# ChrisTho23/DrakeGPT

Measured on AMD Instinct MI355X. Metric: training tokens/sec (fwd+bwd+AdamW), higher is better.
Workload: dtype bf16; 1 GPU; TransformerLM_scaled: V=80 C=384 T=256 heads=6 layers=6 dropout=0.2; fwd+bwd+AdamW; hipGraph=on; batch_per_gpu=64, global_batch=64, seq_len=256, parallelism=dp1, dp_gradient_buckets=1, params=10800464

## Files before the change

### drakegpt_amd/csrc/chain.hip

```cpp
#include "common.h"
#include <stdlib.h>

typedef __attribute__((address_space(1))) const void* gptr_t;
typedef __attribute__((address_space(3))) void* lptr_t;

#define CH_C 384
#define CH_ROWS 64
#define CH_STAGE_B 24576
#define CH_STAGE_A 4096
#define CH_STAGE (CH_STAGE_B + CH_STAGE_A)
#define CH_NST 4
#define CH_ARES (CH_NST * CH_STAGE)
#define CH_KS (CH_C / 32)

struct ChainP {
    const char* o;
    const float* x;
    const char* wproj; const float* bproj;
    float* x1;
    const float* ln2w; const float* ln2b; float* mean2; float* rstd2; bf16_t* h2;
    const char* w1; const float* b1; bf16_t* f; unsigned char* bits;
    const char* w2; const float* b2;
    float* x2; bf16_t* x2b;
    const float* ln1w; const float* ln1b; float* mean1; float* rstd1; bf16_t* h1;
// ... 470 lines not shown
                stamp(4 + 2 * c);
            }
        }
        if (HAS_FFN2) {
            piece(4 * KS, MODE != 4, HAS_QKV, false, true);
            stamp(11);
            if (p.dbg == 4 || p.dbg == 5) { if (LN_FFN2) __builtin_amdgcn_s_barrier(); }
            else {
                float xv[2][3][8];
                residual_epilogue(xv, row0, MODE == 1 ? p.b2 : nullptr, p.x1, key_ffn, MODE != 1 ? p.x2 : nullptr, p.x2b);
                if (LN_FFN2)
                    layernorm(xv, (float*)(lds + (g & (CH_NST - 1)) * CH_STAGE + CH_STAGE_B), row0, p.mean1, p.rstd1, p.h1);
            }
        }
        stamp(12);
        if (HAS_QKV) {
            for (int c = 0; c < 3; ++c) {
                piece(KS, false, c < 2, MODE == 0 && c == 0);
                stamp(13 + 2 * c);
                if (p.dbg == 4 || p.dbg == 5) continue;
                const int lo = opaque_lane(), fr = lo & 15, fg = lo >> 4, col_l = wn * 96 + (fg & 1) * 16 + (fg >> 1) * 8;
#pragma unroll
                for (int q = 0; q < 3; ++q) {
                    const int col = c * C + col_l + 32 * q;
#pragma unroll
                    for (int i = 0; i < 2; ++i) {
                        const int64_t row = row0 + wm * 32 + i * 16 + fr;
                        float v[8];
                        take(i, q, v);
                        bf16x8 o;
#pragma unroll
                        for (int e = 0; e < 8; ++e) o[e] = (bf16_t)v[e];
                        if (p.dbg != 6) *(bf16x8*)(p.qkv + row0 * (3 * C) + mad24(wm * 32 + i * 16 + fr, 3 * C, col)) = o;
                    }
                }
                stamp(14 + 2 * c);
            }
        }
        stamp(19);
        __builtin_amdgcn_s_barrier();
        stamp(20);
    }
}

struct PackOne { const unsigned short* src; unsigned short* dst; int N, K; int64_t ld; };
__global__ __launch_bounds__(256) void pack_chain_kernel(const int64_t* __restrict__ desc, int n_desc, PackOne one) {
    const unsigned short* src = one.src;
    unsigned short* dst = one.dst;
    int K = one.K;
    int64_t ld = one.ld;
    int k = blockIdx.x;
    if (desc) {
        int d = 0;
        for (int i = 1; i < n_desc; ++i)
            if ((int64_t)blockIdx.x >= desc[i * 6 + 4]) d = i;
        const int64_t* D = desc + d * 6;
        src = (const unsigned short*)D[0]; dst = (unsigned short*)D[1]; K = (int)D[3]; ld = D[5];
        k = (int)((int64_t)blockIdx.x - D[4]);
    }
    const int KT = K / 32, c = k / KT, t = k % KT;
    if (!(KT & 1)) {
        const int half = t & 1, t0 = t - half;
        const int64_t k0 = k - half;
#pragma unroll
        for (int u = 0; u < 6; ++u) {
            const int idx = threadIdx.x + 256 * u, line = 96 * half + (idx >> 4), hi = (idx >> 3) & 1, j = idx & 7;
            const int slot = (hi * 4 + (j & 3)) ^ (line & 7);
            const int row = c * 384 + line + 192 * hi, col = t0 * 32 + 8 * j;
            *(u32x4*)(dst + ((k0 + (j >> 2)) * 1536 + line * 8 + slot) * 8) = *(const u32x4*)(src + (int64_t)row * ld + col);
        }
        return;
    }
#pragma unroll
    for (int u = 0; u < 6; ++u) {
        const int idx = threadIdx.x + 256 * u, line = idx >> 3, slot = idx & 7, ls = slot ^ (line & 7);
        const int row = c * 384 + line + 192 * (ls >> 2), col = t * 32 + 8 * (ls & 3);
        *(u32x4*)(dst + ((int64_t)k * 1536 + idx) * 8) = *(const u32x4*)(src + (int64_t)row * ld + col);
    }
}

extern "C" int dg_pack_chain_weights(const void* w, int64_t ld, void* packed, int N, int K, void* stream) {
    if (!w || !packed || N <= 0 || K <= 0 || N % 384 || K % 32 || ld < K || ld % 8 || !dg_aligned16(w) || !dg_aligned16(packed)) return DG_ERR_ARG;
    PackOne one{(const unsigned short*)w, (unsigned short*)packed, N, K, ld};
    hipLaunchKernelGGL(pack_chain_kernel, dim3((N / 384) * (K / 32)), dim3(256), 0, (hipStream_t)stream, (const int64_t*)nullptr, 0, one);
    DG_LAUNCH_CHECK();
    return DG_OK;
}

extern "C" int dg_pack_chain_weights_batched(const int64_t* desc, int n_desc, int total_stages, void* stream) {
    if (!desc || n_desc <= 0 || total_stages <= 0) return DG_ERR_ARG;
    PackOne one{nullptr, nullptr, 0, 0, 0};
    hipLaunchKernelGGL(pack_chain_kernel, dim3(total_stages), dim3(256), 0, (hipStream_t)stream, desc, n_desc, one);
    DG_LAUNCH_CHECK();
    return DG_OK;
}

__global__ __launch_bounds__(256) void l2_warm_kernel(const char* __restrict__ p, int64_t n_lines, float* __restrict__ sink) {
    const int j = (int)blockIdx.x >> 3, per = (int)gridDim.x >> 3;
    float acc = 0.f;
    for (int64_t i = (int64_t)j * 256 + threadIdx.x; i < n_lines; i += (int64_t)per * 256) acc += *(const float*)(p + i * 128);
    if (acc == 123.456f && sink) sink[0] = acc;
}

extern "C" int dg_l2_warm(const void* p, int64_t bytes, void* stream) {
    if (!p || bytes <= 0 || (((uintptr_t)p) & 127)) return DG_ERR_ARG;
    hipLaunchKernelGGL(l2_warm_kernel, dim3(256), dim3(256), 0, (hipStream_t)stream, (const char*)p, bytes / 128, (float*)nullptr);
    DG_LAUNCH_CHECK();
    return DG_OK;
// ... 62 lines not shown
```

### drakegpt_amd/csrc/cross_entropy.hip

```cpp
#include "common.h"
#include <float.h>
#include <type_traits>

struct CeOpt { float eps, zeta; };
struct CeIgn { int64_t ignore_index; const float* inv_count; };
template <typename... O> struct CePack {
    static constexpr bool OPT = dg_pack_has<CeOpt, O...>::value, IGN = dg_pack_has<CeIgn, O...>::value;
    CeOpt opt;
    CeIgn ign;
    __device__ __forceinline__ explicit CePack(O... o) : opt(dg_pack_get(CeOpt{0.f, 0.f}, o...)), ign(dg_pack_get(CeIgn{0, nullptr}, o...)) {}
};
__device__ __forceinline__ float ce_objective(float mx, float logs, float xt, float sd, int V, CeOpt opt) {
    const float lse = mx + logs;
    return logs + (1.f - opt.eps) * (mx - xt) + opt.eps / (float)V * sd + opt.zeta * lse * lse;
}
template <bool OPT, bool IGN>
__device__ __forceinline__ float ce_row_loss(float mx, float logs, float xt, float sd, int V, CeOpt opt) {
    return OPT ? ce_objective(mx, logs, xt, sd, V, opt) : IGN ? logs + (mx - xt) : mx + logs - xt;
}
__device__ __forceinline__ float ce_pscale(float mx, float logs, CeOpt opt) { return 1.f + 2.f * opt.zeta * (mx + logs); }
template <bool OPT> __device__ __forceinline__ float ce_inv(float mx, float logs, float s, CeOpt opt) {
    return OPT ? ce_pscale(mx, logs, opt) / s : 1.f / s;
}
template <bool OPT> __device__ __forceinline__ float ce_unif(int V, CeOpt opt) { return OPT ? opt.eps / (float)V : 0.f; }
// ... 89 lines not shown
    }
    if (!ok) return;
    if (IGN && skip) {
        if (sub == 0) loss_rows[row] = 0.f;
        if (dlogits) {
#pragma unroll
            for (int k = 0; k < 8; ++k)
                if (sub + 16 * k < (int)ldd) dlogits[(int64_t)row * ldd + sub + 16 * k] = from_f32<TD>(0.f);
        }
        return;
    }
    const int64_t t = ce_clamp_target(targets[row], V);
    if (sub == 0) loss_rows[row] = ce_row_loss<OPT, IGN>(mx, logf(s), x[t], sd, V, p.opt);
    if (dlogits) {
        TD* d = dlogits + (int64_t)row * ldd;
        const float inv = ce_inv<OPT>(mx, logf(s), s, p.opt), unif = ce_unif<OPT>(V, p.opt);
        if (gs_dev) grad_scale *= gs_dev[0];
        if (IGN) grad_scale *= p.ign.inv_count[0];
#pragma unroll
        for (int k = 0; k < 8; ++k) {
            const int i = sub + 16 * k;
            if (i < (int)ldd) d[i] = from_f32<TD>(i >= V ? 0.f : ce_grad<OPT>(v[k] * inv, i == (int)t, unif, p.opt, grad_scale));
        }
    }
}

struct CeFuse {
    float* colsum_part; int64_t part_stride; int rows_per;
    float* loss_part; unsigned* counter; float* loss_out; float loss_scale;
};
#define CEF_THREADS 1024
#define CEF_RG (CEF_THREADS / 16)
template <typename TD, typename... O>
__global__ __launch_bounds__(CEF_THREADS) void cross_entropy_small_fused_kernel(const float* __restrict__ logits, int64_t ldl, const int64_t* __restrict__ targets,
                                                                        float* __restrict__ loss_rows, TD* __restrict__ dlogits, int64_t ldd,
                                                                        float grad_scale, int M, int V, CeFuse fz, O... o) {
    const CePack<O...> p(o...);
    constexpr bool OPT = p.OPT, IGN = p.IGN;
    __shared__ float red[CEF_RG][128];
    __shared__ float lred[CEF_RG];
    __shared__ unsigned last_flag;
    const int tid = threadIdx.x, sub = tid & 15, rg = tid >> 4;
    const int m_begin = blockIdx.x * fz.rows_per;
    int m_end = m_begin + fz.rows_per; if (m_end > M) m_end = M;
    float cacc[8];
#pragma unroll
    for (int k = 0; k < 8; ++k) cacc[k] = 0.f;
    float lsum = 0.f;
    if (IGN) grad_scale *= p.ign.inv_count[0];
    for (int r0 = m_begin; r0 < m_end; r0 += CEF_RG) {
        const int row = r0 + rg;
        const bool ok = row < m_end;
        const float* x = logits + (int64_t)(ok ? row : m_begin) * ldl;
        const bool skip = IGN && ok && targets[row] == p.ign.ignore_index;
        float v[8];
        float mx = -INFINITY;
#pragma unroll
        for (int k = 0; k < 8; ++k) {
            const int i = sub + 16 * k;
            v[k] = i < V ? (IGN && skip ? 0.f : x[i]) : -INFINITY;
            mx = fmaxf(mx, v[k]);
        }
#pragma unroll
        for (int o = 8; o > 0; o >>= 1) mx = fmaxf(mx, __shfl_xor(mx, o, 64));
        float s = 0.f, sd = 0.f;
#pragma unroll
        for (int k = 0; k < 8; ++k) {
            if (OPT && sub + 16 * k < V) sd += mx - v[k];
            v[k] = expf(v[k] - mx); s += v[k];
        }
#pragma unroll
        for (int sh = 8; sh > 0; sh >>= 1) s += __shfl_xor(s, sh, 64);
        if (OPT) {
#pragma unroll
            for (int sh = 8; sh > 0; sh >>= 1) sd += __shfl_xor(sd, sh, 64);
        }
        if (!ok) continue;
        if (IGN && skip) {
            if (sub == 0) loss_rows[row] = 0.f;
#pragma unroll
            for (int k = 0; k < 8; ++k)
                if (sub + 16 * k < (int)ldd) dlogits[(int64_t)row * ldd + sub + 16 * k] = from_f32<TD>(0.f);
            continue;
        }
        const int64_t t = ce_clamp_target(targets[row], V);
        const float lr = ce_row_loss<OPT, IGN>(mx, logf(s), x[t], sd, V, p.opt);
        if (sub == 0) { loss_rows[row] = lr; lsum += lr; }
        TD* d = dlogits + (int64_t)row * ldd;
        const float inv = ce_inv<OPT>(mx, logf(s), s, p.opt), unif = ce_unif<OPT>(V, p.opt);
#pragma unroll
        for (int k = 0; k < 8; ++k) {
            const int i = sub + 16 * k;
            const float gk = i >= V ? 0.f : ce_grad<OPT>(v[k] * inv, i == (int)t, unif, p.opt, grad_scale);
            cacc[k] += gk;
            if (i < (int)ldd) d[i] = from_f32<TD>(gk);
        }
    }
#pragma unroll
    for (int k = 0; k < 8; ++k) red[rg][sub + 16 * k] = cacc[k];
    if (sub == 0) lred[rg] = lsum;
    __syncthreads();
    if (fz.colsum_part && tid < V) {
        float c = 0.f;
#pragma unroll 8
        for (int r = 0; r < CEF_RG; ++r) c += red[r][tid];
        fz.colsum_part[(int64_t)blockIdx.x * fz.part_stride + tid] = c;
    }
    if (!fz.loss_out) return;
    if (tid == 0) {
        float b = 0.f;
#pragma unroll 8
        for (int r = 0; r < CEF_RG; ++r) b += lred[r];
        __hip_atomic_store(fz.loss_part + blockIdx.x, b, __ATOMIC_RELAXED, __HIP_MEMORY_SCOPE_AGENT);
        asm volatile("s_waitcnt vmcnt(0)" ::: "memory");
        const unsigned prev = __hip_atomic_fetch_add(fz.counter, 1u, __ATOMIC_RELAXED, __HIP_MEMORY_SCOPE_AGENT);
        last_flag = prev == gridDim.x - 1 ? 1u : 0u;
    }
    __syncthreads();
    if (!last_flag) return;
    __builtin_amdgcn_fence(__ATOMIC_ACQUIRE, "workgroup");
    float* sh = &red[0][0];
    for (int i = tid; i < (int)gridDim.x; i += CEF_THREADS) sh[i] = __hip_atomic_load(fz.loss_part + i, __ATOMIC_RELAXED, __HIP_MEMORY_SCOPE_AGENT);
    __syncthreads();
    if (tid == 0) {
        float tot = 0.f;
        for (int i = 0; i < (int)gridDim.x; ++i) tot += sh[i];
        fz.loss_out[0] = IGN ? tot * (fz.loss_scale * p.ign.inv_count[0]) : tot * fz.loss_scale;
        __hip_atomic_store(fz.counter, 0u, __ATOMIC_RELAXED, __HIP_MEMORY_SCOPE_AGENT);
    }
}

#define CE_BLOCK 1024
#define CE_MAXK 52
__device__ __forceinline__ float ce_block_max(const float* red) {
    __syncthreads();
    float mx = red[0];
#pragma unroll
    for (int k = 1; k < 16; ++k) mx = fmaxf(mx, red[k]);
    __syncthreads();
    return mx;
}
struct CeSums { float s, sd; };
template <bool OPT> __device__ __forceinline__ CeSums ce_block_sums(const float* red, const float* red2) {
    __syncthreads();
    float s = red[0], sd = 0.f;
#pragma unroll
    for (int k = 1; k < 16; ++k) s += red[k];
    if (OPT) {
        sd = red2[0];
#pragma unroll
        for (int k = 1; k < 16; ++k) sd += red2[k];
    }
    return CeSums{s, sd};
}

template <typename TD, typename TL = float, typename... O>
__global__ __launch_bounds__(CE_BLOCK) void cross_entropy_row_kernel(const TL* logits, int64_t ldl, const int64_t* __restrict__ targets,
                                                                      float* __restrict__ loss_rows, TD* dlogits, int64_t ldd,
                                                                      float grad_scale, const float* __restrict__ gs_dev, int M, int V, O... o) {
    const CePack<O...> p(o...);
    constexpr bool OPT = p.OPT, IGN = p.IGN;
    __shared__ float red[16];
    __shared__ float red2[OPT ? 16 : 1];
    const int tid = threadIdx.x, lane = tid & 63, w = tid >> 6;
    const int row = blockIdx.x;
    const TL* x = logits + (int64_t)row * ldl;
    int64_t t = targets[row];
    if (IGN && t == p.ign.ignore_index)
        return ce_zero_row(loss_rows, dlogits, ldd, row, tid, CE_BLOCK);
    float v[CE_MAXK];
    float mx = -INFINITY;
    t = ce_clamp_target(t, V);
    const float xt = (float)x[t];
#pragma unroll
    for (int k = 0; k < CE_MAXK; ++k) {
        const int i = k * CE_BLOCK + tid;
        v[k] = i < V ? (float)x[i] : -INFINITY;
        mx = fmaxf(mx, v[k]);
    }
// ... 280 lines not shown
```

### drakegpt_amd/csrc/elementwise.hip

```cpp
#include "common.h"

__global__ void state_advance_kernel(uint32_t* st) { st[2] += 1u; }

extern "C" int dg_state_advance(uint32_t* rng_state, void* stream) {
    if (!rng_state) return DG_ERR_ARG;
    hipLaunchKernelGGL(state_advance_kernel, dim3(1), dim3(1), 0, (hipStream_t)stream, rng_state);
    DG_LAUNCH_CHECK();
    return DG_OK;
}

__global__ void batch_gather_kernel(const int64_t* __restrict__ corpus, int64_t n_corpus,
                                    const int64_t* __restrict__ off, int64_t* __restrict__ x,
                                    int64_t* __restrict__ y, int B, int T) {
    int64_t i = (int64_t)blockIdx.x * blockDim.x + threadIdx.x;
    if (i >= (int64_t)B * T) return;
    int b = (int)(i / T), t = (int)(i % T);
    int64_t o = off[b] + t;
    int64_t o1 = o + 1;
    if (o < 0) o = 0; if (o >= n_corpus) o = n_corpus - 1;
    if (o1 < 0) o1 = 0; if (o1 >= n_corpus) o1 = n_corpus - 1;
    x[i] = corpus[o];
    y[i] = corpus[o1];
}

// ... 18 lines not shown
    const int cv = C / VEC;
    int64_t total = M * cv;
    const int64_t* off = nullptr;
    if (GATHER) {
        uint32_t row = 0;
        if (bs.ctl) {
            const uint32_t n_rows = bs.ctl[1];
            row = bs.step_state[2] - bs.ctl[0];
            if (row >= n_rows) row = n_rows ? n_rows - 1 : 0;
        }
        off = bs.offsets + (int64_t)row * bs.B;
    }
    (void)total;
    const int lane = threadIdx.x & 63;
    const int64_t wave0 = ((int64_t)blockIdx.x * blockDim.x + threadIdx.x) >> 6, nwaves = ((int64_t)gridDim.x * blockDim.x) >> 6;
    for (int64_t m = wave0; m < M; m += nwaves) {
        const uint32_t mu = (uint32_t)__builtin_amdgcn_readfirstlane((int)m);
        const uint32_t bq = mu / (uint32_t)T;
        const int t = (int)(mu - bq * (uint32_t)T);
        int64_t v;
        if (GATHER) {
            int64_t o = off[bq] + t, o1 = o + 1;
            if (o < 0) o = 0; if (o >= bs.n_corpus) o = bs.n_corpus - 1;
            if (o1 < 0) o1 = 0; if (o1 >= bs.n_corpus) o1 = bs.n_corpus - 1;
            v = bs.corpus[o];
            if (lane == 0) { bs.x_ids[m] = v; bs.y_ids[m] = bs.corpus[o1]; }
        } else {
            v = idx[m];
        }
        v = v < 0 ? 0 : (v >= V ? V - 1 : v);
      for (int j = lane; j < cv; j += 64) {
        const int c = j * VEC;
        if (onehot) {
            if (VEC == 4 && j * 8 < ld_onehot) {
                bf16x8 o;
#pragma unroll
                for (int e = 0; e < 8; ++e) o[e] = (bf16_t)((int64_t)(j * 8 + e) == v ? 1.f : 0.f);
                *(bf16x8*)(onehot + m * ld_onehot + j * 8) = o;
            }
        }
        if (VEC == 4) {
            f32x4 a = *(const f32x4*)(tok + v * C + c);
            if (pos) a += *(const f32x4*)(pos + (int64_t)t * C + c);
            *(f32x4*)(x + m * C + c) = a;
        } else {
            float a = tok[v * C + c];
            if (pos) a += pos[(int64_t)t * C + c];
            x[m * C + c] = a;
        }
      }
    }
}

extern "C" int dg_embed_fwd(const int64_t* idx, const float* tok, const float* pos, float* x,
                            int B, int T, int C, int V, void* onehot, int64_t ld_onehot, void* stream) {
    if (!idx || !tok || !x || B <= 0 || T <= 0 || C <= 0 || V <= 0) return DG_ERR_ARG;
    if (onehot && (C % 4 || ld_onehot % 8 || ld_onehot < V || (int64_t)(C / 4) * 8 < ld_onehot || !dg_aligned16(onehot))) return DG_ERR_ARG;
    int64_t M = (int64_t)B * T;
    bool vec = (C % 4 == 0) && dg_aligned16(tok) && dg_aligned16(x) && (!pos || dg_aligned16(pos));
    int64_t total = vec ? M * (C / 4) : M * C;
    unsigned grid = (unsigned)((total + 255) / 256);
    if (grid > 4096) grid = 4096;
    if (vec)
        hipLaunchKernelGGL(embed_fwd_kernel<4>, dim3(grid), dim3(256), 0, (hipStream_t)stream, idx, tok, pos, x, M, T, C, V, (bf16_t*)onehot, ld_onehot, BatchSrc{});
    else {
        if (onehot) return DG_ERR_ALIGN;
        hipLaunchKernelGGL(embed_fwd_kernel<1>, dim3(grid), dim3(256), 0, (hipStream_t)stream, idx, tok, pos, x, M, T, C, V, (bf16_t*)nullptr, (int64_t)0, BatchSrc{});
    }
    DG_LAUNCH_CHECK();
    return DG_OK;
}

extern "C" int dg_batch_embed_fwd(const int64_t* corpus, int64_t n_corpus, const int64_t* offsets, const uint32_t* step_state,
                                  const uint32_t* ctl, int64_t* x_ids, int64_t* y_ids, const float* tok, const float* pos, float* x,
                                  int B, int T, int C, int V, void* onehot, int64_t ld_onehot, void* stream) {
    if (!corpus || !offsets || !x_ids || !y_ids || !tok || !x || B <= 0 || T <= 0 || C <= 0 || V <= 0 || n_corpus < 2) return DG_ERR_ARG;
    if ((ctl != nullptr) != (step_state != nullptr)) return DG_ERR_ARG;
    if (onehot && (C % 4 || ld_onehot % 8 || ld_onehot < V || (int64_t)(C / 4) * 8 < ld_onehot || !dg_aligned16(onehot))) return DG_ERR_ARG;
    int64_t M = (int64_t)B * T;
    bool vec = (C % 4 == 0) && dg_aligned16(tok) && dg_aligned16(x) && (!pos || dg_aligned16(pos));
    int64_t total = vec ? M * (C / 4) : M * C;
    unsigned grid = (unsigned)((total + 255) / 256);
    if (grid > 4096) grid = 4096;
    const BatchSrc bs{corpus, n_corpus, offsets, step_state, ctl, x_ids, y_ids, B};
    if (vec)
        hipLaunchKernelGGL((embed_fwd_kernel<4, true>), dim3(grid), dim3(256), 0, (hipStream_t)stream, (const int64_t*)nullptr, tok, pos, x, M, T, C, V, (bf16_t*)onehot, ld_onehot, bs);
    else {
        if (onehot) return DG_ERR_ALIGN;
        hipLaunchKernelGGL((embed_fwd_kernel<1, true>), dim3(grid), dim3(256), 0, (hipStream_t)stream, (const int64_t*)nullptr, tok, pos, x, M, T, C, V, (bf16_t*)nullptr, (int64_t)0, bs);
    }
    DG_LAUNCH_CHECK();
    return DG_OK;
}

__global__ void embed_window_kernel(const int64_t* __restrict__ ids, int64_t ld_ids, const uint32_t* __restrict__ state,
                                    const float* __restrict__ tok, const float* __restrict__ pos, float* __restrict__ x,
                                    int B, int Tw, int C, int V, int mode) {
    const int64_t L = (int64_t)state[2];
    if (L < 1 || L > ld_ids || (mode == 0 ? L > Tw : L < Tw)) return;
    const int rows_per_b = mode == 0 ? 1 : Tw;
    const int lane = threadIdx.x & 63;
    const int64_t wave0 = ((int64_t)blockIdx.x * blockDim.x + threadIdx.x) >> 6, nwaves = ((int64_t)gridDim.x * blockDim.x) >> 6;
    const int64_t Mrows = (int64_t)B * rows_per_b;
    for (int64_t m = wave0; m < Mrows; m += nwaves) {
        const int b = (int)(m / rows_per_b), i = (int)(m % rows_per_b);
        const int64_t col = mode == 0 ? L - 1 : L - Tw + i;
        const int t = mode == 0 ? (int)(L - 1) : i;
        int64_t v = ids[(int64_t)b * ld_ids + col];
        v = v < 0 ? 0 : (v >= V ? V - 1 : v);
        for (int c = lane; c < C; c += 64) x[m * C + c] = tok[v * C + c] + pos[(int64_t)t * C + c];
    }
}

extern "C" int dg_embed_window(const int64_t* ids, int64_t ld_ids, const uint32_t* state, const float* tok, const float* pos,
                               float* x, int B, int Tw, int C, int V, int mode, void* stream) {
    if (!ids || !state || !tok || !pos || !x || ld_ids <= 0 || B <= 0 || Tw <= 0 || C <= 0 || V <= 0 || (mode != 0 && mode != 1))
        return DG_ERR_ARG;
    const int64_t rows = (int64_t)B * (mode == 0 ? 1 : Tw);
    unsigned grid = (unsigned)((rows + 3) / 4);
    if (grid > 4096) grid = 4096;
    hipLaunchKernelGGL(embed_window_kernel, dim3(grid), dim3(256), 0, (hipStream_t)stream, ids, ld_ids, state, tok, pos, x, B, Tw, C, V, mode);
    DG_LAUNCH_CHECK();
    return DG_OK;
}

__global__ void zero_f32_kernel(float* __restrict__ p, int64_t n) {
    const int64_t n4 = n / 4;
    for (int64_t i = (int64_t)blockIdx.x * blockDim.x + threadIdx.x; i < n4; i += (int64_t)gridDim.x * blockDim.x)
        ((f32x4*)p)[i] = (f32x4){0.f, 0.f, 0.f, 0.f};
    for (int64_t i = n4 * 4 + (int64_t)blockIdx.x * blockDim.x + threadIdx.x; i < n; i += (int64_t)gridDim.x * blockDim.x) p[i] = 0.f;
}

template <typename TX>
__global__ void embed_bwd_tok_kernel(const int64_t* __restrict__ idx, const TX* __restrict__ dx,
                                     float* __restrict__ dtok, int64_t M, int C, int V) {
    int64_t total = M * C;
    for (int64_t i = (int64_t)blockIdx.x * blockDim.x + threadIdx.x; i < total;
         i += (int64_t)gridDim.x * blockDim.x) {
        int64_t m = i / C;
        int c = (int)(i % C);
        int64_t v = idx[m];
        v = v < 0 ? 0 : (v >= V ? V - 1 : v);
        atomicAdd(dtok + v * C + c, (float)dx[i]);
    }
}
template <typename TX>
__global__ __launch_bounds__(256) void embed_bwd_pos_kernel(const TX* __restrict__ dx, float* __restrict__ dpos,
                                                            int B, int T, int C) {
    __shared__ f32x4 red[4][64];
    const int64_t tc = (int64_t)T * C;
    const int lane = threadIdx.x & 63, g = threadIdx.x >> 6;
    const int64_t i = ((int64_t)blockIdx.x * 64 + lane) * 4;
    const bool vec = (tc % 4 == 0);
    f32x4 s = {0.f, 0.f, 0.f, 0.f};
    if (i < tc) {
        if (vec) {
            typedef TX TX4 __attribute__((ext_vector_type(4)));
            for (int b = g; b < B; b += 4) {
                const TX4 t = *(const TX4*)(dx + (int64_t)b * tc + i);
                s += (f32x4){(float)t[0], (float)t[1], (float)t[2], (float)t[3]};
            }
        } else {
            for (int b = g; b < B; b += 4)
#pragma unroll
                for (int e = 0; e < 4; ++e)
                    if (i + e < tc) s[e] += (float)dx[(int64_t)b * tc + i + e];
        }
    }
    red[g][lane] = s;
    __syncthreads();
    if (g == 0 && i < tc) {
        const f32x4 t = (red[0][lane] + red[1][lane]) + (red[2][lane] + red[3][lane]);
#pragma unroll
        for (int e = 0; e < 4; ++e)
            if (i + e < tc) dpos[i + e] = t[e];
    }
}
extern "C" int dg_embed_bwd(const int64_t* idx, const void* dx_v, int dx_dtype, float* dtok, float* dpos,
                            int B, int T, int C, int V, void* stream) {
    if (dx_dtype != DG_F32 && dx_dtype != DG_BF16) return DG_ERR_DTYPE;
    const float* dx = (const float*)dx_v;
    if (!idx || !dx || (!dtok && !dpos) || B <= 0 || T <= 0 || C <= 0 || V <= 0) return DG_ERR_ARG;
    hipStream_t s = (hipStream_t)stream;
    int64_t M = (int64_t)B * T;
    if (dtok) {
        const int64_t nz = (int64_t)V * C;
        if (!dg_aligned16(dtok)) return DG_ERR_ALIGN;
        unsigned zgrid = (unsigned)((nz / 4 + 255) / 256);
        if (zgrid < 1) zgrid = 1; if (zgrid > 4096) zgrid = 4096;
        hipLaunchKernelGGL(zero_f32_kernel, dim3(zgrid), dim3(256), 0, s, dtok, nz);
        DG_LAUNCH_CHECK();
        int64_t total = M * C;
        unsigned grid = (unsigned)((total + 255) / 256);
        if (grid > 8192) grid = 8192;
        if (dx_dtype == DG_BF16) hipLaunchKernelGGL(embed_bwd_tok_kernel<bf16_t>, dim3(grid), dim3(256), 0, s, idx, (const bf16_t*)dx_v, dtok, M, C, V);
        else hipLaunchKernelGGL(embed_bwd_tok_kernel<float>, dim3(grid), dim3(256), 0, s, idx, dx, dtok, M, C, V);
        DG_LAUNCH_CHECK();
    }
    if (dpos) {
        int64_t tc = (int64_t)T * C;
        if (dx_dtype == DG_BF16)
            hipLaunchKernelGGL(embed_bwd_pos_kernel<bf16_t>, dim3((unsigned)((tc + 255) / 256)), dim3(256), 0, s, (const bf16_t*)dx_v, dpos, B, T, C);
        else
            hipLaunchKernelGGL(embed_bwd_pos_kernel<float>, dim3((unsigned)((tc + 255) / 256)), dim3(256), 0, s, dx, dpos, B, T, C);
        DG_LAUNCH_CHECK();
    }
    return DG_OK;
}

template <typename TI, typename TO>
__global__ void cast_kernel(const TI* __restrict__ in, TO* __restrict__ out, int64_t n) {
    int64_t stride = (int64_t)gridDim.x * blockDim.x;
    int64_t n4 = n / 4;
    for (int64_t i = (int64_t)blockIdx.x * blockDim.x + threadIdx.x; i < n4; i += stride) {
        float v[4];
#pragma unroll
        for (int j = 0; j < 4; ++j) v[j] = to_f32<TI>(in[i * 4 + j]);
#pragma unroll
        for (int j = 0; j < 4; ++j) out[i * 4 + j] = from_f32<TO>(v[j]);
    }
    for (int64_t i = n4 * 4 + (int64_t)blockIdx.x * blockDim.x + threadIdx.x; i < n; i += stride)
        out[i] = from_f32<TO>(to_f32<TI>(in[i]));
}

extern "C" int dg_cast(const void* in, int in_dtype, void* out, int out_dtype, int64_t n, void* stream) {
    if (!in || !out || n < 0) return DG_ERR_ARG;
    if (n == 0) return DG_OK;
    unsigned grid = (unsigned)((n / 4 + 255) / 256);
    if (grid == 0) grid = 1;
    if (grid > 4096) grid = 4096;
    hipStream_t s = (hipStream_t)stream;
    if (in_dtype == DG_F32 && out_dtype == DG_BF16)
        hipLaunchKernelGGL((cast_kernel<float, bf16_t>), dim3(grid), dim3(256), 0, s, (const float*)in, (bf16_t*)out, n);
    else if (in_dtype == DG_BF16 && out_dtype == DG_F32)
        hipLaunchKernelGGL((cast_kernel<bf16_t, float>), dim3(grid), dim3(256), 0, s, (const bf16_t*)in, (float*)out, n);
    else if (in_dtype == DG_F32 && out_dtype == DG_F32)
        hipLaunchKernelGGL((cast_kernel<float, float>), dim3(grid), dim3(256), 0, s, (const float*)in, (float*)out, n);
    else
        return DG_ERR_DTYPE;
    DG_LAUNCH_CHECK();
    return DG_OK;
}

template <typename TO>
__global__ void transpose_cast_kernel(const float* __restrict__ in, int64_t ldi, TO* __restrict__ out,
                                      int64_t ldo, int R, int Cc) {
    __shared__ float tile[64][65];
    int r0 = blockIdx.y * 64, c0 = blockIdx.x * 64;
    int tx = threadIdx.x & 63, ty = threadIdx.x >> 6;
    for (int i = ty; i < 64; i += 4) {
        int r = r0 + i, c = c0 + tx;
        tile[i][tx] = (r < R && c < Cc) ? in[(int64_t)r * ldi + c] : 0.f;
    }
    __syncthreads();
    for (int i = ty; i < 64; i += 4) {
        int c = c0 + i, r = r0 + tx;
        if (c < Cc && r < ldo) out[(int64_t)c * ldo + r] = from_f32<TO>(tile[tx][i]);
    }
}

extern "C" int dg_transpose_cast(const float* in, int64_t ldi, void* out, int64_t ldo, int dtype,
                                 int R, int Cc, void* stream) {
    if (!in || !out || R <= 0 || Cc <= 0 || ldi < Cc || ldo < R) return DG_ERR_ARG;
    dim3 grid((Cc + 63) / 64, (unsigned)((ldo + 63) / 64));
    if (dtype == DG_BF16)
        hipLaunchKernelGGL(transpose_cast_kernel<bf16_t>, grid, dim3(256), 0, (hipStream_t)stream, in, ldi, (bf16_t*)out, ldo, R, Cc);
    else if (dtype == DG_F32)
        hipLaunchKernelGGL(transpose_cast_kernel<float>, grid, dim3(256), 0, (hipStream_t)stream, in, ldi, (float*)out, ldo, R, Cc);
    else
        return DG_ERR_DTYPE;
    DG_LAUNCH_CHECK();
    return DG_OK;
}

template <typename TI, typename TO>
__global__ void transpose_cast_batched_kernel(const int64_t* __restrict__ desc, int n_desc) {
    __shared__ float tile[64][65];
    int d = 0;
    for (int i = 1; i < n_desc; ++i)
        if ((int64_t)blockIdx.x >= desc[i * 8 + 6]) d = i;
    const int64_t* D = desc + d * 8;
    const TI* in = (const TI*)D[0];
    TO* out = (TO*)D[1];
    const int64_t ldi = D[2], ldo = D[3];
    const int R = (int)D[4], Cc = (int)D[5];
    const int local = (int)((int64_t)blockIdx.x - D[6]), tiles_x = (int)D[7];
    const int r0 = (local / tiles_x) * 64, c0 = (local % tiles_x) * 64;
    const int tx = threadIdx.x & 63, ty = threadIdx.x >> 6;
    for (int i = ty; i < 64; i += 4) {
        int r = r0 + i, c = c0 + tx;
        tile[i][tx] = (r < R && c < Cc) ? to_f32<TI>(in[(int64_t)r * ldi + c]) : 0.f;
    }
    __syncthreads();
    for (int i = ty; i < 64; i += 4) {
        int c = c0 + i, r = r0 + tx;
        if (c < Cc && r < ldo) out[(int64_t)c * ldo + r] = from_f32<TO>(tile[tx][i]);
    }
}

__global__ __launch_bounds__(256) void transpose_bf16_batched_kernel(const int64_t* __restrict__ desc, int n_desc) {
    constexpr int PITCH = 68;
    __shared__ __attribute__((aligned(16))) unsigned short tile[64 * PITCH];
    int d = 0;
    for (int i = 1; i < n_desc; ++i)
        if ((int64_t)blockIdx.x >= desc[i * 8 + 6]) d = i;
    const int64_t* D = desc + d * 8;
    const unsigned short* in = (const unsigned short*)D[0];
    unsigned short* out = (unsigned short*)D[1];
    const int64_t ldi = D[2], ldo = D[3];
    const int R = (int)D[4], Cc = (int)D[5];
    const int local = (int)((int64_t)blockIdx.x - D[6]), tiles_x = (int)D[7];
    const int r0 = (local / tiles_x) * 64, c0 = (local % tiles_x) * 64;
    const bool vec = ((ldi | ldo) % 8 == 0) && ((((uintptr_t)in) | ((uintptr_t)out)) % 16 == 0);
#pragma unroll
    for (int pass = 0; pass < 2; ++pass) {
        const int pc = threadIdx.x + 256 * pass, row = pc >> 3, ck = pc & 7;
        const int r = r0 + row, c = c0 + 8 * ck;
        u32x4 v = {0u, 0u, 0u, 0u};
        if (r < R) {
            const unsigned short* src = in + (int64_t)r * ldi + c;
            if (vec && c + 8 <= Cc) v = *(const u32x4*)src;
            else {
                unsigned short e[8];
#pragma unroll
                for (int j = 0; j < 8; ++j) e[j] = (c + j < Cc) ? src[j] : (unsigned short)0;
                v = (u32x4){e[0] | ((uint32_t)e[1] << 16), e[2] | ((uint32_t)e[3] << 16), e[4] | ((uint32_t)e[5] << 16), e[6] | ((uint32_t)e[7] << 16)};
            }
        }
        uint2* dst = (uint2*)(tile + row * PITCH + 8 * ck);
        dst[0] = make_uint2(v[0], v[1]);
        dst[1] = make_uint2(v[2], v[3]);
    }
    __syncthreads();
#pragma unroll
    for (int pass = 0; pass < 2; ++pass) {
        const int pc = threadIdx.x + 256 * pass, oc = (pc & 7) + 8 * (pc >> 6), rk = (pc >> 3) & 7;
        const int c = c0 + oc, r = r0 + 8 * rk;
        if (c >= Cc || r >= ldo) continue;
        unsigned short e[8];
#pragma unroll
        for (int j = 0; j < 8; ++j) e[j] = tile[(8 * rk + j) * PITCH + oc];
        unsigned short* dstp = out + (int64_t)c * ldo + r;
        if (vec && r + 8 <= ldo)
            *(u32x4*)dstp = (u32x4){e[0] | ((uint32_t)e[1] << 16), e[2] | ((uint32_t)e[3] << 16), e[4] | ((uint32_t)e[5] << 16), e[6] | ((uint32_t)e[7] << 16)};
        else {
#pragma unroll
            for (int j = 0; j < 8; ++j)
                if (r + j < ldo) dstp[j] = e[j];
        }
    }
}

__global__ __launch_bounds__(256) void transpose_u8_batched_kernel(const int64_t* __restrict__ desc, int n_desc) {
    constexpr int PITCH = 144;
    __shared__ __attribute__((aligned(16))) unsigned char ta[128 * PITCH], tb[128 * PITCH];
    int d = 0;
    for (int i = 1; i < n_desc; ++i)
        if ((int64_t)blockIdx.x >= desc[i * 8 + 6]) d = i;
// ... 277 lines not shown
#pragma unroll
        for (int j = 0; j < 8; ++j) {
            const int cc = lane * 8 + j;
            if (c + j < N) o[j] = red[0][cc] + red[1][cc] + red[2][cc] + red[3][cc];
        }
    }
}

extern "C" int dg_colsum(const void* A, int64_t lda, int dtype, float* part, int64_t part_stride,
                         int n_partials, int M, int N, void* stream) {
    if (!A || !part || M <= 0 || N <= 0 || n_partials <= 0) return DG_ERR_ARG;
    int rows_per = rows_per_partial(M, n_partials);
    dim3 grid(n_partials, (N + 255) / 256), block(256);
    hipStream_t s = (hipStream_t)stream;
    if (dtype == DG_BF16 && lda % 8 == 0 && lda >= (N + 7) / 8 * 8 && dg_aligned16(A)) {
        hipLaunchKernelGGL(colsum_bf16_kernel, dim3(n_partials, (N + 511) / 512), dim3(256), 0, s, (const bf16_t*)A, lda, M, N, part,
                           part_stride, rows_per);
        DG_LAUNCH_CHECK();
        return DG_OK;
    }
    if (dtype == DG_BF16)
        hipLaunchKernelGGL((dropbwd_cast_kernel<bf16_t, float, false>), grid, block, 0, s, (const bf16_t*)A, lda, (float*)nullptr, (int64_t)0, M, N, 1.f, 0u, (const uint32_t*)nullptr, 0u, (const float*)nullptr, (int64_t)0, part, part_stride, rows_per);
    else if (dtype == DG_F32)
        hipLaunchKernelGGL((dropbwd_cast_kernel<float, float, false>), grid, block, 0, s, (const float*)A, lda, (float*)nullptr, (int64_t)0, M, N, 1.f, 0u, (const uint32_t*)nullptr, 0u, (const float*)nullptr, (int64_t)0, part, part_stride, rows_per);
    else return DG_ERR_DTYPE;
    DG_LAUNCH_CHECK();
    return DG_OK;
}

__global__ void reduce_partials_kernel(const float* __restrict__ part, int64_t stride, int n_partials,
                                       float* __restrict__ out, int64_t n, int vec_ok) {
    int64_t gs = (int64_t)gridDim.x * blockDim.x;
    if (vec_ok) {
        int64_t n4 = n / 4;
        for (int64_t i = (int64_t)blockIdx.x * blockDim.x + threadIdx.x; i < n4; i += gs) {
            f32x4 s = ((const f32x4*)part)[i];
            for (int g = 1; g < n_partials; ++g) s += *(const f32x4*)(part + (int64_t)g * stride + i * 4);
            ((f32x4*)out)[i] = s;
        }
        for (int64_t i = n4 * 4 + (int64_t)blockIdx.x * blockDim.x + threadIdx.x; i < n; i += gs) {
            float s = part[i];
            for (int g = 1; g < n_partials; ++g) s += part[(int64_t)g * stride + i];
            out[i] = s;
        }
    } else {
        for (int64_t i = (int64_t)blockIdx.x * blockDim.x + threadIdx.x; i < n; i += gs) {
            float s = part[i];
            for (int g = 1; g < n_partials; ++g) s += part[(int64_t)g * stride + i];
            out[i] = s;
        }
    }
}

__global__ __launch_bounds__(1024) void reduce_partials_tall_kernel(const float* __restrict__ part, int64_t stride, int n_partials,
                                                                    float* __restrict__ out, int64_t n4) {
    __shared__ f32x4 red[16][64];
    const int c = threadIdx.x & 63, r = threadIdx.x >> 6;
    const int64_t i = (int64_t)blockIdx.x * 64 + c;
    f32x4 s0 = {0.f, 0.f, 0.f, 0.f}, s1 = s0;
    if (i < n4) {
        int g = r;
        for (; g + 16 < n_partials; g += 32) {
            s0 += *(const f32x4*)(part + (int64_t)g * stride + i * 4);
            s1 += *(const f32x4*)(part + (int64_t)(g + 16) * stride + i * 4);
        }
        if (g < n_partials) s0 += *(const f32x4*)(part + (int64_t)g * stride + i * 4);
    }
    red[r][c] = s0 + s1;
    __syncthreads();
    if (r == 0 && i < n4) {
        f32x4 t = red[0][c];
#pragma unroll
        for (int k = 1; k < 16; ++k) t += red[k][c];
        ((f32x4*)out)[i] = t;
    }
}

extern "C" int dg_reduce_partials(const float* partials, int64_t stride, int n_partials,
                                  float* out, int64_t n, void* stream) {
    if (!partials || !out || n_partials <= 0 || n < 0) return DG_ERR_ARG;
    if (n == 0) return DG_OK;
    int vec_ok = dg_aligned16(partials) && dg_aligned16(out) && (stride % 4 == 0);
    if (vec_ok && n_partials >= 32 && n % 4 == 0 && n / 4 < (int64_t)n_partials * 4096) {
        const int64_t n4 = n / 4;
        hipLaunchKernelGGL(reduce_partials_tall_kernel, dim3((unsigned)((n4 + 63) / 64)), dim3(1024), 0, (hipStream_t)stream,
                           partials, stride, n_partials, out, n4);
        DG_LAUNCH_CHECK();
        return DG_OK;
    }
    int64_t work = vec_ok ? (n + 3) / 4 : n;
    unsigned grid = (unsigned)((work + 255) / 256);
    if (grid > 4096) grid = 4096;
    hipLaunchKernelGGL(reduce_partials_kernel, dim3(grid), dim3(256), 0, (hipStream_t)stream, partials, stride, n_partials, out, n, vec_ok);
    DG_LAUNCH_CHECK();
    return DG_OK;
}

__device__ __forceinline__ float reduce_sum_factor(float scale) { return scale; }
__device__ __forceinline__ float reduce_sum_factor(float scale, const float* scale_dev) { return scale * scale_dev[0]; }
template <typename... S>
__global__ void reduce_sum_kernel(const float* __restrict__ x, int64_t n, float scale, S... scale_dev, float* __restrict__ out) {
    __shared__ float red[16];
    float s = 0.f;
    for (int64_t i = threadIdx.x; i < n; i += 1024) s += x[i];
    s = wave_sum(s);
    if ((threadIdx.x & 63) == 0) red[threadIdx.x >> 6] = s;
    __syncthreads();
    if (threadIdx.x < 64) {
        float t = threadIdx.x < 16 ? red[threadIdx.x] : 0.f;
        t = wave_sum(t);
        if (threadIdx.x == 0) out[0] = t * reduce_sum_factor(scale, scale_dev...);
    }
}

extern "C" int dg_reduce_sum(const float* x, int64_t n, float scale, float* out, void* stream) {
    if (!x || !out || n <= 0) return DG_ERR_ARG;
    hipLaunchKernelGGL(reduce_sum_kernel<>, dim3(1), dim3(1024), 0, (hipStream_t)stream, x, n, scale, out);
    DG_LAUNCH_CHECK();
    return DG_OK;
}

extern "C" int dg_reduce_sum_scaled(const float* x, int64_t n, float scale, const float* scale_dev, float* out, void* stream) {
    if (!x || !out || !scale_dev || n <= 0) return DG_ERR_ARG;
    hipLaunchKernelGGL(reduce_sum_kernel<const float* __restrict__>, dim3(1), dim3(1024), 0, (hipStream_t)stream, x, n, scale, scale_dev, out);
    DG_LAUNCH_CHECK();
    return DG_OK;
}

__global__ void softmax_rows_kernel(const float* __restrict__ logits, int64_t ldl, float* __restrict__ probs,
                                    int64_t ldp, int M, int V) {
    int row = blockIdx.x * (blockDim.x >> 6) + (threadIdx.x >> 6);
    int lane = threadIdx.x & 63;
    if (row >= M) return;
    const float* x = logits + (int64_t)row * ldl;
    float mx = -INFINITY;
    for (int i = lane; i < V; i += 64) mx = fmaxf(mx, x[i]);
    mx = wave_max(mx);
    float s = 0.f;
// ... 257 lines not shown
```

Before: 7.138 million tokens/s.

## Tune small auxiliary kernels: ballot descriptor lookup, embed rows4, pos-grad, reductions

Several independent micro-optimizations land together. Descriptor lookup in the pack and transpose kernels now uses a wave ballot instead of a serial loop. Cross-entropy takes the target logit from registers and batches its shared-memory reductions. A new embedding forward kernel handles four rows per wave, and a new bf16x8 vectorized kernel computes the positional gradient. The tall partial-reduce kernel changes to smaller blocks with deeper unrolled loads. These mainly cut latency in small kernels, and they add more code paths that need alignment and size guards.

After: 7.182 million tokens/s (median of 6 runs). No clear change (+0.6%).

```diff
diff --git a/drakegpt_amd/csrc/chain.hip b/drakegpt_amd/csrc/chain.hip
--- a/drakegpt_amd/csrc/chain.hip
+++ b/drakegpt_amd/csrc/chain.hip
@@ -546,8 +546,15 @@
     int k = blockIdx.x;
     if (desc) {
         int d = 0;
-        for (int i = 1; i < n_desc; ++i)
-            if ((int64_t)blockIdx.x >= desc[i * 6 + 4]) d = i;
+        if (n_desc <= 64) {
+            const int lane = threadIdx.x & 63;
+            const bool at = lane >= 1 && lane < n_desc && (int64_t)blockIdx.x >= desc[lane * 6 + 4];
+            const unsigned long long mask = __ballot(at);
+            d = mask ? 63 - __builtin_clzll(mask) : 0;
+        } else {
+            for (int i = 1; i < n_desc; ++i)
+                if ((int64_t)blockIdx.x >= desc[i * 6 + 4]) d = i;
+        }
         const int64_t* D = desc + d * 6;
         src = (const unsigned short*)D[0]; dst = (unsigned short*)D[1]; K = (int)D[3]; ld = D[5];
         k = (int)((int64_t)blockIdx.x - D[4]);
diff --git a/drakegpt_amd/csrc/cross_entropy.hip b/drakegpt_amd/csrc/cross_entropy.hip
--- a/drakegpt_amd/csrc/cross_entropy.hip
+++ b/drakegpt_amd/csrc/cross_entropy.hip
@@ -165,7 +165,8 @@
         const int row = r0 + rg;
         const bool ok = row < m_end;
         const float* x = logits + (int64_t)(ok ? row : m_begin) * ldl;
-        const bool skip = IGN && ok && targets[row] == p.ign.ignore_index;
+        const int64_t tg = ok ? targets[row] : 0;
+        const bool skip = IGN && ok && tg == p.ign.ignore_index;
         float v[8];
         float mx = -INFINITY;
 #pragma unroll
@@ -174,6 +175,12 @@
             v[k] = i < V ? (IGN && skip ? 0.f : x[i]) : -INFINITY;
             mx = fmaxf(mx, v[k]);
         }
+        const int64_t t = ce_clamp_target(tg, V);
+        float xt = 0.f;
+#pragma unroll
+        for (int k = 0; k < 8; ++k)
+            if (sub + 16 * k == (int)t) xt = v[k];
+        xt = __shfl(xt, (int)t & 15, 16);
 #pragma unroll
         for (int o = 8; o > 0; o >>= 1) mx = fmaxf(mx, __shfl_xor(mx, o, 64));
         float s = 0.f, sd = 0.f;
@@ -196,8 +203,7 @@
                 if (sub + 16 * k < (int)ldd) dlogits[(int64_t)row * ldd + sub + 16 * k] = from_f32<TD>(0.f);
             continue;
         }
-        const int64_t t = ce_clamp_target(targets[row], V);
-        const float lr = ce_row_loss<OPT, IGN>(mx, logf(s), x[t], sd, V, p.opt);
+        const float lr = ce_row_loss<OPT, IGN>(mx, logf(s), xt, sd, V, p.opt);
         if (sub == 0) { loss_rows[row] = lr; lsum += lr; }
         TD* d = dlogits + (int64_t)row * ldd;
         const float inv = ce_inv<OPT>(mx, logf(s), s, p.opt), unif = ce_unif<OPT>(V, p.opt);
@@ -214,16 +220,22 @@
     if (sub == 0) lred[rg] = lsum;
     __syncthreads();
     if (fz.colsum_part && tid < V) {
+        float q[CEF_RG];
+#pragma unroll
+        for (int r = 0; r < CEF_RG; ++r) q[r] = red[r][tid];
         float c = 0.f;
-#pragma unroll 8
-        for (int r = 0; r < CEF_RG; ++r) c += red[r][tid];
+#pragma unroll
+        for (int r = 0; r < CEF_RG; ++r) c += q[r];
         fz.colsum_part[(int64_t)blockIdx.x * fz.part_stride + tid] = c;
     }
     if (!fz.loss_out) return;
-    if (tid == 0) {
+    if (tid == CEF_THREADS - 64) {
+        float q[CEF_RG];
+#pragma unroll
+        for (int r = 0; r < CEF_RG; ++r) q[r] = lred[r];
         float b = 0.f;
-#pragma unroll 8
-        for (int r = 0; r < CEF_RG; ++r) b += lred[r];
+#pragma unroll
+        for (int r = 0; r < CEF_RG; ++r) b += q[r];
         __hip_atomic_store(fz.loss_part + blockIdx.x, b, __ATOMIC_RELAXED, __HIP_MEMORY_SCOPE_AGENT);
         asm volatile("s_waitcnt vmcnt(0)" ::: "memory");
         const unsigned prev = __hip_atomic_fetch_add(fz.counter, 1u, __ATOMIC_RELAXED, __HIP_MEMORY_SCOPE_AGENT);
@@ -237,7 +249,16 @@
     __syncthreads();
     if (tid == 0) {
         float tot = 0.f;
-        for (int i = 0; i < (int)gridDim.x; ++i) tot += sh[i];
+        const int n = (int)gridDim.x;
+        int i = 0;
+        for (; i + 64 <= n; i += 64) {
+            float q[64];
+#pragma unroll
+            for (int j = 0; j < 64; ++j) q[j] = sh[i + j];
+#pragma unroll
+            for (int j = 0; j < 64; ++j) tot += q[j];
+        }
+        for (; i < n; ++i) tot += sh[i];
         fz.loss_out[0] = IGN ? tot * (fz.loss_scale * p.ign.inv_count[0]) : tot * fz.loss_scale;
         __hip_atomic_store(fz.counter, 0u, __ATOMIC_RELAXED, __HIP_MEMORY_SCOPE_AGENT);
     }
diff --git a/drakegpt_amd/csrc/elementwise.hip b/drakegpt_amd/csrc/elementwise.hip
--- a/drakegpt_amd/csrc/elementwise.hip
+++ b/drakegpt_amd/csrc/elementwise.hip
@@ -94,6 +94,93 @@
     }
 }
 
+__global__ __launch_bounds__(256) void embed_fwd_rows4_kernel(const float* __restrict__ tok, const float* __restrict__ pos, float* __restrict__ x,
+                                                              int64_t M, int T, int C, int V, bf16_t* __restrict__ onehot, int64_t ld_onehot,
+                                                              BatchSrc bs) {
+    const int cv = C / 4;
+    uint32_t row = 0;
+    if (bs.ctl) {
+        const uint32_t n_rows = bs.ctl[1];
+        row = bs.step_state[2] - bs.ctl[0];
+        if (row >= n_rows) row = n_rows ? n_rows - 1 : 0;
+    }
+    const int64_t* off = bs.offsets + (int64_t)row * bs.B;
+    const int lane = threadIdx.x & 63;
+    const int64_t wave0 = ((int64_t)blockIdx.x * blockDim.x + threadIdx.x) >> 6, nwaves = ((int64_t)gridDim.x * blockDim.x) >> 6;
+    for (int64_t m0 = wave0 * 4; m0 < M; m0 += nwaves * 4) {
+        const uint32_t m0u = (uint32_t)__builtin_amdgcn_readfirstlane((int)m0);
+        int vi;
+        {
+            const uint32_t ml = m0u + (uint32_t)(lane & 3);
+            const bool in = (int64_t)ml < M;
+            const uint32_t mc = in ? ml : (uint32_t)(M - 1);
+            const uint32_t bq = mc / (uint32_t)T;
+            const int t = (int)(mc - bq * (uint32_t)T);
+            int64_t o = off[bq] + t, o1 = o + 1;
+            if (o < 0) o = 0; if (o >= bs.n_corpus) o = bs.n_corpus - 1;
+            if (o1 < 0) o1 = 0; if (o1 >= bs.n_corpus) o1 = bs.n_corpus - 1;
+            const int64_t v = bs.corpus[o];
+            if (lane < 4 && in) { bs.x_ids[mc] = v; bs.y_ids[mc] = bs.corpus[o1]; }
+            vi = (int)(v < 0 ? 0 : (v >= V ? V - 1 : v));
+        }
+        int vr[4], tr[4];
+        bool okr[4];
+#pragma unroll
+        for (int r = 0; r < 4; ++r) {
+            vr[r] = __builtin_amdgcn_readlane(vi, r);
+            const uint32_t mu = m0u + (uint32_t)r;
+            okr[r] = (int64_t)mu < M;
+            tr[r] = (int)(mu % (uint32_t)T);
+        }
+        f32x4 a[4][2];
+#pragma unroll
+        for (int r = 0; r < 4; ++r)
+#pragma unroll
+            for (int k = 0; k < 2; ++k) {
+                const int j = lane + 64 * k;
+                if (okr[r] && j < cv) a[r][k] = *(const f32x4*)(tok + (int64_t)vr[r] * C + j * 4);
+            }
+        if (pos) {
+            f32x4 p[4][2];
+#pragma unroll
+            for (int r = 0; r < 4; ++r)
+#pragma unroll
+                for (int k = 0; k < 2; ++k) {
+                    const int j = lane + 64 * k;
+                    if (okr[r] && j < cv) p[r][k] = *(const f32x4*)(pos + (int64_t)tr[r] * C + j * 4);
+                }
+#pragma unroll
+            for (int r = 0; r < 4; ++r)
+#pragma unroll
+                for (int k = 0; k < 2; ++k) {
+                    const int j = lane + 64 * k;
+                    if (okr[r] && j < cv) a[r][k] += p[r][k];
+                }
+        }
+#pragma unroll
+        for (int r = 0; r < 4; ++r) {
+            if (!okr[r]) continue;
+            const int64_t m = (int64_t)m0u + r;
+#pragma unroll
+            for (int k = 0; k < 2; ++k) {
+                const int j = lane + 64 * k;
+                if (j >= cv) continue;
+                if (onehot && j * 8 < ld_onehot) {
+                    bf16x8 o;
+#pragma unroll
+                    for (int e = 0; e < 8; ++e) o[e] = (bf16_t)(j * 8 + e == vr[r] ? 1.f : 0.f);
+                    *(bf16x8*)(onehot + m * ld_onehot + j * 8) = o;
+                }
+                *(f32x4*)(x + m * C + j * 4) = a[r][k];
+            }
+        }
+    }
+}
+static inline unsigned embed_rows4_grid(int64_t M) {
+    const int64_t g = (M + 15) / 16;
+    return (unsigned)(g > 4096 ? 4096 : g);
+}
+
 extern "C" int dg_embed_fwd(const int64_t* idx, const float* tok, const float* pos, float* x,
                             int B, int T, int C, int V, void* onehot, int64_t ld_onehot, void* stream) {
     if (!idx || !tok || !x || B <= 0 || T <= 0 || C <= 0 || V <= 0) return DG_ERR_ARG;
@@ -125,7 +212,9 @@
     unsigned grid = (unsigned)((total + 255) / 256);
     if (grid > 4096) grid = 4096;
     const BatchSrc bs{corpus, n_corpus, offsets, step_state, ctl, x_ids, y_ids, B};
-    if (vec)
+    if (vec && C <= 512 && M < ((int64_t)1 << 31))
+        hipLaunchKernelGGL(embed_fwd_rows4_kernel, dim3(embed_rows4_grid(M)), dim3(256), 0, (hipStream_t)stream, tok, pos, x, M, T, C, V, (bf16_t*)onehot, ld_onehot, bs);
+    else if (vec)
         hipLaunchKernelGGL((embed_fwd_kernel<4, true>), dim3(grid), dim3(256), 0, (hipStream_t)stream, (const int64_t*)nullptr, tok, pos, x, M, T, C, V, (bf16_t*)onehot, ld_onehot, bs);
     else {
         if (onehot) return DG_ERR_ALIGN;
@@ -216,6 +305,53 @@
 #pragma unroll
         for (int e = 0; e < 4; ++e)
             if (i + e < tc) dpos[i + e] = t[e];
+    }
+}
+__global__ __launch_bounds__(64) void embed_bwd_pos_bf16x8_kernel(const bf16_t* __restrict__ dx, float* __restrict__ dpos, int B, int64_t tc) {
+    __shared__ __attribute__((aligned(16))) float red[4][16][8];
+    const int l = threadIdx.x & 15, g = threadIdx.x >> 4;
+    const int64_t i = ((int64_t)blockIdx.x * 16 + l) * 8;
+    float s[8];
+#pragma unroll
+    for (int e = 0; e < 8; ++e) s[e] = 0.f;
+    if (i < tc) {
+        const bf16_t* col = dx + i;
+        int b = g;
+        for (; b + 60 < B; b += 64) {
+            bf16x8 t[16];
+#pragma unroll
+            for (int u = 0; u < 16; ++u) t[u] = *(const bf16x8*)(col + (int64_t)(b + 4 * u) * tc);
+#pragma unroll
+            for (int u = 0; u < 16; ++u)
+#pragma unroll
+                for (int e = 0; e < 8; ++e) s[e] += (float)t[u][e];
+        }
+        for (; b + 12 < B; b += 16) {
+            bf16x8 t[4];
+#pragma unroll
+            for (int u = 0; u < 4; ++u) t[u] = *(const bf16x8*)(col + (int64_t)(b + 4 * u) * tc);
+#pragma unroll
+            for (int u = 0; u < 4; ++u)
+#pragma unroll
+                for (int e = 0; e < 8; ++e) s[e] += (float)t[u][e];
+        }
+        for (; b < B; b += 4) {
+            const bf16x8 t = *(const bf16x8*)(col + (int64_t)b * tc);
+#pragma unroll
+            for (int e = 0; e < 8; ++e) s[e] += (float)t[e];
+        }
+    }
+#pragma unroll
+    for (int e = 0; e < 8; ++e) red[g][l][e] = s[e];
+    __syncthreads();
+    if (g == 0 && i < tc) {
+#pragma unroll
+        for (int h = 0; h < 2; ++h) {
+            f32x4 o;
+#pragma unroll
+            for (int e = 0; e < 4; ++e) o[e] = (red[0][l][4 * h + e] + red[1][l][4 * h + e]) + (red[2][l][4 * h + e] + red[3][l][4 * h + e]);
+            *(f32x4*)(dpos + i + 4 * h) = o;
+        }
     }
 }
 extern "C" int dg_embed_bwd(const int64_t* idx, const void* dx_v, int dx_dtype, float* dtok, float* dpos,
@@ -241,7 +377,9 @@
     }
     if (dpos) {
         int64_t tc = (int64_t)T * C;
-        if (dx_dtype == DG_BF16)
+        if (dx_dtype == DG_BF16 && tc % 8 == 0 && dg_aligned16(dx_v) && dg_aligned16(dpos))
+            hipLaunchKernelGGL(embed_bwd_pos_bf16x8_kernel, dim3((unsigned)((tc + 127) / 128)), dim3(64), 0, s, (const bf16_t*)dx_v, dpos, B, tc);
+        else if (dx_dtype == DG_BF16)
             hipLaunchKernelGGL(embed_bwd_pos_kernel<bf16_t>, dim3((unsigned)((tc + 255) / 256)), dim3(256), 0, s, (const bf16_t*)dx_v, dpos, B, T, C);
         else
             hipLaunchKernelGGL(embed_bwd_pos_kernel<float>, dim3((unsigned)((tc + 255) / 256)), dim3(256), 0, s, dx, dpos, B, T, C);
@@ -340,12 +478,23 @@
     }
 }
 
+__device__ __forceinline__ int desc_of_tile(const int64_t* __restrict__ desc, int n_desc, int64_t tile) {
+    if (n_desc <= 64) {
+        const int lane = threadIdx.x & 63;
+        const bool at = lane >= 1 && lane < n_desc && tile >= desc[lane * 8 + 6];
+        const unsigned long long m = __ballot(at);
+        return m ? 63 - __builtin_clzll(m) : 0;
+    }
+    int d = 0;
+    for (int i = 1; i < n_desc; ++i)
+        if (tile >= desc[i * 8 + 6]) d = i;
+    return d;
+}
+
 __global__ __launch_bounds__(256) void transpose_bf16_batched_kernel(const int64_t* __restrict__ desc, int n_desc) {
     constexpr int PITCH = 68;
     __shared__ __attribute__((aligned(16))) unsigned short tile[64 * PITCH];
-    int d = 0;
-    for (int i = 1; i < n_desc; ++i)
-        if ((int64_t)blockIdx.x >= desc[i * 8 + 6]) d = i;
+    const int d = desc_of_tile(desc, n_desc, (int64_t)blockIdx.x);
     const int64_t* D = desc + d * 8;
     const unsigned short* in = (const unsigned short*)D[0];
     unsigned short* out = (unsigned short*)D[1];
@@ -729,14 +878,25 @@
     }
 }
 
-__global__ __launch_bounds__(1024) void reduce_partials_tall_kernel(const float* __restrict__ part, int64_t stride, int n_partials,
-                                                                    float* __restrict__ out, int64_t n4) {
-    __shared__ f32x4 red[16][64];
-    const int c = threadIdx.x & 63, r = threadIdx.x >> 6;
-    const int64_t i = (int64_t)blockIdx.x * 64 + c;
+#define RPT_COLS 16
+__global__ __launch_bounds__(16 * RPT_COLS) void reduce_partials_tall_kernel(const float* __restrict__ part, int64_t stride, int n_partials,
+                                                                             float* __restrict__ out, int64_t n4) {
+    __shared__ f32x4 red[16][RPT_COLS];
+    const int c = threadIdx.x & (RPT_COLS - 1), r = threadIdx.x / RPT_COLS;
+    const int64_t i = (int64_t)blockIdx.x * RPT_COLS + c;
     f32x4 s0 = {0.f, 0.f, 0.f, 0.f}, s1 = s0;
     if (i < n4) {
         int g = r;
+        for (; g + 16 + 7 * 32 < n_partials; g += 8 * 32) {
+            f32x4 a[8], b[8];
+#pragma unroll
+            for (int u = 0; u < 8; ++u) {
+                a[u] = *(const f32x4*)(part + (int64_t)(g + 32 * u) * stride + i * 4);
+                b[u] = *(const f32x4*)(part + (int64_t)(g + 32 * u + 16) * stride + i * 4);
+            }
+#pragma unroll
+            for (int u = 0; u < 8; ++u) { s0 += a[u]; s1 += b[u]; }
+        }
         for (; g + 16 < n_partials; g += 32) {
             s0 += *(const f32x4*)(part + (int64_t)g * stride + i * 4);
             s1 += *(const f32x4*)(part + (int64_t)(g + 16) * stride + i * 4);
@@ -758,9 +918,9 @@
     if (!partials || !out || n_partials <= 0 || n < 0) return DG_ERR_ARG;
     if (n == 0) return DG_OK;
     int vec_ok = dg_aligned16(partials) && dg_aligned16(out) && (stride % 4 == 0);
-    if (vec_ok && n_partials >= 32 && n % 4 == 0 && n / 4 < (int64_t)n_partials * 4096) {
+    if (vec_ok && n_partials >= 32 && n % 4 == 0 && n / 4 < (int64_t)n_partials * 4096 && n / 4 / RPT_COLS < 0x7fffffff) {
         const int64_t n4 = n / 4;
-        hipLaunchKernelGGL(reduce_partials_tall_kernel, dim3((unsigned)((n4 + 63) / 64)), dim3(1024), 0, (hipStream_t)stream,
+        hipLaunchKernelGGL(reduce_partials_tall_kernel, dim3((unsigned)((n4 + RPT_COLS - 1) / RPT_COLS)), dim3(16 * RPT_COLS), 0, (hipStream_t)stream,
                            partials, stride, n_partials, out, n4);
         DG_LAUNCH_CHECK();
         return DG_OK;
```
